# IlyaGrebnov/libbsc

Measured on AMD Instinct MI355X. Metric: MB/s compress (BWT+QLFC) on 64 MiB blocks, higher is better.
Workload: dtype u8; 1 GPU; 1 x 64 MiB synth-text-v1 block(s) per step, bsc_compress(lzp off, sorter=1, coder=1); 5 GPU context(s) x 4 block(s) in flight per GPU, 20 coder threads; block_bytes=67108864, sorter=BWT, coder=QLFC static (-e1), parallelism=block-parallel x1, compressed_bytes_rank0=15277890

## Files before the change

include/bscgpu.h:

```cpp
#ifndef BSCGPU_H
#define BSCGPU_H

#include <stddef.h>
#include <stdint.h>

#if defined(__GNUC__)
#define BSCGPU_API __attribute__((visibility("default")))
#else
#define BSCGPU_API
#endif

#ifdef __cplusplus
extern "C" {
#endif

typedef struct bscgpu_ctx bscgpu_ctx;

BSCGPU_API int bscgpu_device_count(void);

BSCGPU_API int  bscgpu_create(bscgpu_ctx** ctx, int device, int64_t max_n);
BSCGPU_API void bscgpu_destroy(bscgpu_ctx* ctx);

BSCGPU_API int64_t bscgpu_arena_bytes(const bscgpu_ctx* ctx);

// ... 160 lines not shown
};
typedef struct bscgpu_kstat {
    double   ms;
    uint64_t launches;
    uint64_t bytes;
    uint64_t records;
} bscgpu_kstat;
BSCGPU_API void bscgpu_profile_enable(bscgpu_ctx* ctx, int on);
BSCGPU_API void bscgpu_profile_reset(bscgpu_ctx* ctx);
BSCGPU_API int  bscgpu_profile_get(bscgpu_ctx* ctx, bscgpu_kstat* stats );
BSCGPU_API int  bscgpu_profile_scatter_launches(bscgpu_ctx* ctx, double* ms, uint64_t* records, int max);
BSCGPU_API int  bscgpu_last_stage_ms(bscgpu_ctx* ctx, double* out6);

BSCGPU_API const char* bscgpu_last_error(const bscgpu_ctx* ctx);

enum { BSCGPU_OPT_RS_ONESWEEP = 1, BSCGPU_CNT_OS_RETRIES = 2, BSCGPU_OPT_DC_PACKED_STREAM = 4,
       BSCGPU_CNT_DC_REPLAYS = 5, BSCGPU_CNT_DC_LAST_FAIL = 6, BSCGPU_CNT_DC_AVG_UNDECIDED = 7, BSCGPU_CNT_DC_HIST_EXTENDED = 8,
       BSCGPU_OPT_BATCH_FRONT = 9, BSCGPU_CNT_BATCH_FRONT_PASSES = 10, BSCGPU_CNT_BATCH_L_PASSES = 11,
       BSCGPU_OPT_DEVICE_RC = 12, BSCGPU_CNT_DEVICE_RC_BLOCKS = 13,
       BSCGPU_OPT_BATCH_MODEL = 14, BSCGPU_CNT_BATCH_MODEL_PASSES = 15, BSCGPU_CNT_BATCH_MODEL_DECLINED = 16,
       BSCGPU_OPT_BATCH_MODEL_FAST = 17, BSCGPU_CNT_BATCH_FAST_PASSES = 18, BSCGPU_CNT_BATCH_FAST_DECLINED = 19,
       BSCGPU_OPT_BWT_FOLD = 20, BSCGPU_CNT_BWT_FOLDED = 21,
       BSCGPU_OPT_BATCH_MODEL_SEGMENTS = 22, BSCGPU_CNT_BATCH_SEGMENTS = 23, BSCGPU_CNT_BATCH_SEG_RERUNS = 24,
       BSCGPU_CNT_BATCH_SEG_HOST_BLOCKS = 25, BSCGPU_CNT_DC_DCAP = 26 };
enum { BSCGPU_DC_FAIL_AVG = 2, BSCGPU_DC_FAIL_HIST = 4, BSCGPU_DC_FAIL_CAP = 8, BSCGPU_DC_FAIL_REPLAY = 16 };
BSCGPU_API int bscgpu_option_set(bscgpu_ctx* ctx, int key, int value);
BSCGPU_API int bscgpu_option_get(bscgpu_ctx* ctx, int key);
enum { BSCGPU_PCNT_DEVICE_MODEL_BLOCKS = 1, BSCGPU_PCNT_REDONE_ON_HOST_MODEL = 2, BSCGPU_PCNT_DEVICE_MODEL_LZP_BLOCKS = 3 };
BSCGPU_API long long bscgpu_process_counter(int key);

BSCGPU_API int bscgpu_dispatch_device(int slot, int nphys);
BSCGPU_API int bscgpu_dispatch_pick(int nphys, int ctx_per_dev, const int* users, const unsigned char* usable, unsigned start);

#ifdef __cplusplus
}
#endif
#endif
```

libbsc_amd/csrc/device/context.hip:

```cpp
#include "dev_common.h"
#include "dma_copy.h"
#include <sys/mman.h>
#include <system_error>
#include <thread>
#include <vector>
#include <chrono>
#include <cstdio>
#include <cstdlib>
#include <cstring>
#include <functional>
#include <memory>
#include <mutex>

int ctx_fail(bscgpu_ctx* c, int code, const char* what, hipError_t e)
{
    if (c) {
        char buf[512];
        snprintf(buf, sizeof buf, "%s: %s", what, e == hipSuccess ? "failed" : hipGetErrorString(e));
        c->err = buf;
    }
    return code;
}

bool ctx_timing_on() { static const bool on = getenv("BSCGPU_TIMING") != nullptr; return on; }
// ... 134 lines not shown
    if (hipGetDeviceCount(&n) != hipSuccess) return 0;
    return n;
}

#ifndef ARENA_ALIGN
#define ARENA_ALIGN 256
#endif
extern "C" int bscgpu_create(bscgpu_ctx** out, int device, int64_t max_n)
{
    if (!out || max_n < 0 || max_n >= 0x7fffffffll) return BSC_BAD_PARAMETER;
    *out = nullptr;
    CtxTimer tm_all("bscgpu_create");
    int ndev = 0;
    if (hipGetDeviceCount(&ndev) != hipSuccess || ndev <= 0) return BSC_GPU_NOT_SUPPORTED;
    if (device < 0 || device >= ndev) return BSC_BAD_PARAMETER;
    devcoder_warm_tables();
    if (hipSetDevice(device) != hipSuccess) return BSC_GPU_ERROR;
    if (!getenv("BSCGPU_SPIN")) { (void)hipSetDeviceFlags(hipDeviceScheduleBlockingSync); (void)hipGetLastError(); }

    bscgpu_ctx* c = new bscgpu_ctx();
    { CtxTimer tm("  first HIP call on this thread"); (void)hipFree(nullptr); }
    c->device = device;
    c->max_n  = max_n;
    { const char* e = getenv("BSC_PS13"); c->dc_p13 = (e && e[0] == '0') ? 0 : 1; }
    { const char* e = getenv("BSC_BWT_FOLD"); if (e && e[0] >= '0' && e[0] <= '2' && !e[1]) c->bwt_fold = e[0] - '0'; }
    memset(c->kstat, 0, sizeof c->kstat);
    auto tm_streams = std::make_unique<CtxTimer>("  streams + events");
    if (hipStreamCreateWithFlags(&c->stream, hipStreamNonBlocking) != hipSuccess) { delete c; return BSC_GPU_ERROR; }
    if (hipEventCreateWithFlags(&c->sync_ev, hipEventBlockingSync | hipEventDisableTiming) != hipSuccess) { hipStreamDestroy(c->stream); delete c; return BSC_GPU_ERROR; }
    if (hipStreamCreateWithFlags(&c->copy_stream, hipStreamNonBlocking) != hipSuccess) { hipEventDestroy(c->sync_ev); hipStreamDestroy(c->stream); delete c; return BSC_GPU_ERROR; }

    tm_streams.reset();
    const size_t N = align_up((size_t)max_n + 4096, 4096);
    struct Carve { void** p; size_t bytes; size_t lead; };
    Carve carve[] = {
        {(void**)&c->dT,      N + 128, 64},
        {(void**)&c->dL,      N + 64, 0},
        {(void**)&c->kA,      8 * N, 0}, {(void**)&c->kB, 8 * N, 0},
        {(void**)&c->vA,      4 * N, 0}, {(void**)&c->vB, 4 * N, 0},
        {(void**)&c->SA,      4 * N, 0}, {(void**)&c->ISA, 4 * N + 64, 0},
        {(void**)&c->cpos[0], 4 * N, 0}, {(void**)&c->cpos[1], 4 * N, 0},
        {(void**)&c->csa[0],  4 * N, 0}, {(void**)&c->csa[1],  4 * N, 0},
        {(void**)&c->cgrp[0], 4 * N, 0}, {(void**)&c->cgrp[1], 4 * N, 0},
        {(void**)&c->flags,   N + 64, 0},
        {(void**)&c->counts,  (size_t)256 * MAX_CHUNKS * 4, 0},
        {(void**)&c->rowtot,  256 * 4, 0},
// ... 106 lines not shown
{
    if (!c) return;
    memset(c->kstat, 0, sizeof c->kstat);
    c->scatter_log.clear();
}
extern "C" int bscgpu_profile_get(bscgpu_ctx* c, bscgpu_kstat* stats)
{
    if (!c || !stats) return BSC_BAD_PARAMETER;
    memcpy(stats, c->kstat, sizeof c->kstat);
    return BSC_NO_ERROR;
}
extern "C" int bscgpu_profile_scatter_launches(bscgpu_ctx* c, double* ms, uint64_t* records, int max)
{
    if (!c) return 0;
    int cnt = (int)c->scatter_log.size();
    int from = cnt > max ? cnt - max : 0;
    for (int i = from; i < cnt; ++i) { ms[i - from] = c->scatter_log[i].ms; records[i - from] = c->scatter_log[i].records; }
    return cnt - from;
}
extern "C" int bscgpu_option_set(bscgpu_ctx* c, int key, int value)
{
    if (!c) return BSC_BAD_PARAMETER;
    if (key == BSCGPU_OPT_RS_ONESWEEP && value >= 0 && value <= 3 && (value == 0 || c->os_available)) { const int old = c->os_mode; c->os_mode = value; return old; }
    if (key == BSCGPU_OPT_DC_PACKED_STREAM && (value == 0 || value == 1)) { const int old = c->dc_p13; c->dc_p13 = value; return old; }
    if (key == BSCGPU_OPT_BATCH_FRONT && (value == 0 || value == 1)) { const int old = c->batch_front; c->batch_front = value; return old; }
    if (key == BSCGPU_OPT_DEVICE_RC && (value == 0 || value == 1)) { const int old = c->device_rc; c->device_rc = value; return old; }
    if (key == BSCGPU_OPT_BATCH_MODEL && (value == 0 || value == 1)) { const int old = c->batch_model; c->batch_model = value; return old; }
    if (key == BSCGPU_OPT_BATCH_MODEL_FAST && (value == 0 || value == 1)) { const int old = c->batch_model_fast; c->batch_model_fast = value; return old; }
    if (key == BSCGPU_OPT_BATCH_MODEL_SEGMENTS && (value == 0 || value == 1)) { const int old = c->batch_model_segments; c->batch_model_segments = value; return old; }
    if (key == BSCGPU_OPT_BWT_FOLD && value >= 0 && value <= 2) { const int old = c->bwt_fold; c->bwt_fold = value; return old; }
    return BSC_BAD_PARAMETER;
}
extern "C" int bscgpu_option_get(bscgpu_ctx* c, int key)
{
    if (!c) return BSC_BAD_PARAMETER;
    if (key == BSCGPU_OPT_RS_ONESWEEP) return c->os_mode;
    if (key == BSCGPU_CNT_OS_RETRIES) return c->os_retries;
    if (key == BSCGPU_OPT_DC_PACKED_STREAM) return c->dc_p13;
    if (key == BSCGPU_CNT_DC_REPLAYS) return c->dc_replays;
    if (key == BSCGPU_CNT_DC_LAST_FAIL) return c->dc_last_fail;
    if (key == BSCGPU_CNT_DC_AVG_UNDECIDED) return c->dc_avg_und;
    if (key == BSCGPU_CNT_DC_HIST_EXTENDED) return c->dc_hist_ext;
    if (key == BSCGPU_OPT_BATCH_FRONT) return c->batch_front;
    if (key == BSCGPU_CNT_BATCH_FRONT_PASSES) return c->cnt_front_passes;
    if (key == BSCGPU_CNT_BATCH_L_PASSES) return c->cnt_l_passes;
    if (key == BSCGPU_OPT_DEVICE_RC) return c->device_rc;
    if (key == BSCGPU_CNT_DEVICE_RC_BLOCKS) return c->cnt_device_rc;
    if (key == BSCGPU_OPT_BATCH_MODEL) return c->batch_model;
    if (key == BSCGPU_CNT_BATCH_MODEL_PASSES) return c->cnt_model_passes;
    if (key == BSCGPU_CNT_BATCH_MODEL_DECLINED) return c->cnt_model_declined;
    if (key == BSCGPU_OPT_BATCH_MODEL_FAST) return c->batch_model_fast;
    if (key == BSCGPU_CNT_BATCH_FAST_PASSES) return c->cnt_model_fast_passes;
    if (key == BSCGPU_CNT_BATCH_FAST_DECLINED) return c->cnt_model_fast_declined;
    if (key == BSCGPU_OPT_BATCH_MODEL_SEGMENTS) return c->batch_model_segments;
    if (key == BSCGPU_CNT_BATCH_SEGMENTS) return c->cnt_seg;
    if (key == BSCGPU_CNT_BATCH_SEG_RERUNS) return c->cnt_seg_reruns;
    if (key == BSCGPU_CNT_BATCH_SEG_HOST_BLOCKS) return c->cnt_seg_host_blocks;
    if (key == BSCGPU_CNT_DC_DCAP) { const int64_t v = devcoder_dcap(c); return v > 0x7fffffff ? 0x7fffffff : (int)v; }
    if (key == BSCGPU_OPT_BWT_FOLD) return c->bwt_fold;
    if (key == BSCGPU_CNT_BWT_FOLDED) return c->cnt_bwt_folded;
    return BSC_BAD_PARAMETER;
}
extern "C" int bscgpu_last_stage_ms(bscgpu_ctx* c, double* out6)
{
    if (!c || !out6) return BSC_BAD_PARAMETER;
// ... 92 lines not shown
```

libbsc_amd/csrc/device/dev_common.h:

```cpp
#pragma once
#include <hip/hip_runtime.h>
#include <stdint.h>
#include <stddef.h>
#include <string>
#include <vector>

#include "../../../include/bscgpu.h"

typedef unsigned long long u64;
typedef unsigned int       u32;
typedef unsigned short     u16;
typedef unsigned char      u8;

#define BSC_NO_ERROR                0
#define BSC_BAD_PARAMETER          -1
#define BSC_NOT_ENOUGH_MEMORY      -2
#define BSC_NOT_COMPRESSIBLE       -3
#define BSC_NOT_SUPPORTED          -4
#define BSC_DATA_CORRUPT           -6
#define BSC_GPU_ERROR              -7
#define BSC_GPU_NOT_SUPPORTED      -8
#define BSC_GPU_NOT_ENOUGH_MEMORY  -9

constexpr int   WG          = 256;
// ... 80 lines not shown
    int  device_rc = 0;
    int  cnt_device_rc = 0;
    int  batch_model = 0;
    int  cnt_model_passes = 0, cnt_model_declined = 0;
    int  batch_model_fast = 0;
    int  cnt_model_fast_passes = 0, cnt_model_fast_declined = 0;
    int  batch_model_segments = 0;
    int  cnt_seg = 0, cnt_seg_reruns = 0, cnt_seg_host_blocks = 0;
    u16* model_host[2] = {nullptr, nullptr};
    size_t model_host_entries = 0;
    bool model_host_failed = false;
    u64* wc_sink = nullptr;
    int  num_cus = 256;
    int  os_mode = 0;
    u32* os_agg = nullptr;
    u32* os_zero = nullptr;
    u32  os_tiles_cap = 0;
    u32  os_pass_stride = 0;
    u32  os_batch_words = 0;
    u32  os_epoch = 0;
    bool os_check_pending = false;
    bool os_available = true;
    int  os_retries = 0;
    int  dc_p13 = 1;
    bool os_gave_up = false;
    int  bwt_fold = 1;
    int  cnt_bwt_folded = 0;
    bool fold_lds_set = false;
    u32* hscal  = nullptr;
    u64* hscal64 = nullptr;
    u64* hadler = nullptr;
    u64* hsplit = nullptr;
    HostSlot slots[MAX_SLOTS];
    int      nslots = 0;
    DevCoder* dc = nullptr;
    bool     dc_alloc_failed = false;
    int      dc_last_fail = 0;
    int      dc_replays = 0;
    int      dc_avg_und = 0;
    int      dc_hist_ext = 0;

    bool         prof        = false;
    bscgpu_kstat kstat[BSCGPU_K_COUNT];
    std::vector<ScatterLaunch> scatter_log;
    struct Pending { hipEvent_t a, b; int kind; u64 bytes; u64 records; };
    std::vector<Pending> pending;
    std::vector<hipEvent_t> event_pool;
    double       stage_ms[6] = {0, 0, 0, 0, 0, 0};

    std::string  err;
};

int  ctx_fail(bscgpu_ctx* c, int code, const char* what, hipError_t e);
bool ctx_timing_on();
struct CtxTimer {
    const char* what; double t0; bool on;
    explicit CtxTimer(const char* w);
    ~CtxTimer();
};
hipError_t ctx_sync(bscgpu_ctx* c);
#define HIP_TRY(ctx, expr)                                                         \
    do { hipError_t _e = (expr);                                                   \
// ... 145 lines not shown
```

libbsc_amd/csrc/device/devcoder.hip:

```cpp
#include "dev_common.h"
#include "dma_copy.h"
#include <thread>
#include <system_error>
#include "devcoder_model.h"
#include "../host/qlfc.h"
#include <cstdio>
#include <cstdlib>
#include <cstring>
#include <deque>
#include <vector>
#include <type_traits>

using namespace dcm;

#ifndef DC_XCD_RANGES
#define DC_XCD_RANGES 0
#endif
__device__ __forceinline__ u32 dc_virtual_block() {
    if (!DC_XCD_RANGES) return blockIdx.x;
    return (blockIdx.x & 7u) * (gridDim.x >> 3) + (blockIdx.x >> 3);
}

constexpr int DC_WCH_MAX  = 4096;
constexpr u32 DC_SIGMASK  = 0x7ffu;
constexpr int DC_ROWS     = 1088;

enum { DM_FAIL = 0, DM_NTYPES, DM_NROUNDS, DM_AVG_UND, DM_REPLAYS, DM_D0, DM_D1, DM_D2, DM_D3, DM_HIST_EXT , DM_P13_OVER , DM_COUNT = 16 };
enum { FAIL_AVG = BSCGPU_DC_FAIL_AVG, FAIL_HIST = BSCGPU_DC_FAIL_HIST, FAIL_CAP = BSCGPU_DC_FAIL_CAP, FAIL_REPLAY = BSCGPU_DC_FAIL_REPLAY };

struct DcSub { u32 nb; u32 first[9]; u32 maxr[8]; };
struct DcRowBins { u16 lo1, hi1, lo2, hi2; };

struct DevCoder {
    size_t Mcap = 0, Dcap = 0;
    char*  arena = nullptr; size_t arena_bytes = 0;
    u64 *key_ch = nullptr, *key_ch_s = nullptr, *key_sr = nullptr, *key_sr_s = nullptr, *key_sn = nullptr, *key_sn_s = nullptr;
    u32 *inv_ch = nullptr, *inv_sr = nullptr, *inv_sn = nullptr;
    u8  *ge32 = nullptr;
    u32 *doff[4] = {nullptr, nullptr, nullptr, nullptr};
    u16 *events[4] = {nullptr, nullptr, nullptr, nullptr};
    u32 *pos[4] = {nullptr, nullptr, nullptr, nullptr};
    u16 *V[4] = {nullptr, nullptr, nullptr, nullptr};
    size_t nch_cap = 0;
    u16 *ps[2] = {nullptr, nullptr};
    u32 *cnt = nullptr, *rowtot = nullptr, *rowstart = nullptr , *wdec = nullptr, *wdecoff = nullptr;
    u16 *elo = nullptr, *ehi = nullptr, *S = nullptr;
    u32 *present = nullptr; u8 *rounds = nullptr; u32 *meta = nullptr; u32 *poff = nullptr;
    DcRowBins* rowbins = nullptr;
    u16* sink = nullptr;
    u8  *tab_rank = nullptr, *tab_run = nullptr;
    ModelParams* mp = nullptr;
    ModelParams* mp_fast = nullptr;
    struct DcFrag* frag = nullptr;
    u32 *hmeta = nullptr;
    char*  batch_arena = nullptr; size_t batch_bytes = 0; bool batch_alloc_failed = false;
    u16 *esub[4] = {nullptr, nullptr, nullptr, nullptr};
    u8  *sub_maxr = nullptr; u32 *poff_tab = nullptr;
    u32 *sub_und = nullptr, *sub_dec = nullptr, *seg_run = nullptr;
    hipEvent_t seg_ev[2] = {nullptr, nullptr};
};

__device__ __forceinline__ u32 dc_sb_of(u32 j, const DcSub& S)
{
    u32 sb = 0;
#pragma unroll
    for (int b = 1; b < 8; ++b) if ((u32)b < S.nb && j >= S.first[b]) sb = b;
    return sb;
}
__device__ __forceinline__ u32 dc_maxr_pack(const DcSub& S)
// ... 615 lines not shown
#pragma unroll
    for (u32 x = 0; x < 8; ++x) {
        const u32 id = (w[x >> 1] >> (16u * (x & 1u))) & 0xffffu;
        if (id != prev && k0 + x < E) ev[k0 + x] |= (u16)DC_ROWMARK;
        prev = id;
    }
}

__device__ __forceinline__ int dc_class_first_row(int cls)
{
    return cls == CLS_RF ? TAU_RF : cls == CLS_RE ? TAU_RE : cls == CLS_RM ? TAU_RM : cls == CLS_RP ? TAU_RP : cls == CLS_NF ? TAU_NF
         : cls == CLS_NE ? TAU_NE : cls == CLS_NM ? TAU_NM : cls == CLS_NM2 ? TAU_NM2 : DC_ROWS;
}

constexpr int DC_EVAL_WAVES = 4;
constexpr int DC_EVAL_LDS_WAVE = 2 * 64 * DC_EROW;
constexpr int DC_EVAL_LDS = DC_EVAL_WAVES * (DC_EVAL_LDS_WAVE + NUM_CLS * 4 + NUM_CLS * (int)sizeof(Rates));
__device__ __forceinline__ void dc_wave_sync()
{
    __builtin_amdgcn_fence(__ATOMIC_ACQ_REL, "wavefront");
    __builtin_amdgcn_wave_barrier();
}

template <bool WRITE>
__global__ __launch_bounds__(64 * DC_EVAL_WAVES) void dc_eval_wave_kernel(DcEvalAll A, const ModelParams* __restrict__ mp, const u32* __restrict__ meta,
                                                          u16* __restrict__ elo_all, u16* __restrict__ ehi_all, const u16* __restrict__ Sv_all, u32* __restrict__ tdbg)
{
#if DC_EVAL_TIMING
    const u64 t_begin = wall_clock64();
    u32 slow_batches = 0;
#endif
    extern __shared__ __attribute__((aligned(16))) u8 dc_eval_lds[];
    const u32 wv = threadIdx.x >> 6, lane = threadIdx.x & 63u;
    u8* const sin = dc_eval_lds + wv * DC_EVAL_LDS_WAVE;
    u8* const sout = sin + 64 * DC_EROW;
    u32* const sclsend = reinterpret_cast<u32*>(dc_eval_lds + DC_EVAL_WAVES * DC_EVAL_LDS_WAVE) + wv * NUM_CLS;
    Rates* const srate = reinterpret_cast<Rates*>(dc_eval_lds + DC_EVAL_WAVES * (DC_EVAL_LDS_WAVE + NUM_CLS * 4)) + wv * NUM_CLS;
    const u32 gw = blockIdx.x * DC_EVAL_WAVES + wv;
    if (meta[DM_FAIL] != 0u || gw >= A.wstart[4]) return;
    int jb = 0;
#pragma unroll
    for (int q = 1; q < 4; ++q) if (gw >= A.wstart[q]) jb = q;
    const DcEvalJob J = A.job[jb];
    if (lane < (u32)NUM_CLS) {
        srate[lane] = mp->rates[lane][J.fam];
        sclsend[lane] = J.rowstart[dc_class_first_row((int)lane + 1)];
    }
    dc_wave_sync();
    u16* const elo = elo_all + A.cstart[jb];
    u16* const ehi = ehi_all + A.cstart[jb];
    const u16* const Sv = Sv_all + A.cstart[jb];
    u16* const Vout = A.V[jb];
    const u32 wave = gw - A.wstart[jb];
    const u32 c = wave * 64 + lane;
    const u32 EV = A.ev;
    const u64 k0 = (u64)c * EV;
    const bool mine = k0 < J.E;
    const u32 k1 = mine ? (u32)((k0 + EV < J.E) ? k0 + EV : J.E) : 0u;
    const u32 crow = lane >> 3, ccol = lane & 7u;
    const u64 wave_k0 = (u64)wave * 64 * EV;

    u32 cls = 0, clsend = 0, prev = 0xffffu;
    int init = mp->init[0];
    int lo = init, hi = init;
    Rates R = srate[0];
    if (mine) {
        while (cls + 1 < (u32)NUM_CLS && sclsend[cls] <= (u32)k0) ++cls;
        clsend = sclsend[cls];
        R = srate[cls];
        init = mp->init[cls];
        prev = (k0 > 0) ? ((u32)J.events[k0 - 1] & DC_SIGMASK) : 0xffffu;
        if (WRITE) { lo = Sv[c]; hi = lo; } else { lo = mp->vmin[cls][J.fam]; hi = mp->vmax[cls][J.fam]; }
    }
    auto fetch = [&](u32 b, uint4* q) {
#pragma unroll
        for (int i = 0; i < 8; ++i) {
            const u64 kk = wave_k0 + (u64)(8 * i + crow) * EV + (u64)b * DC_EB + ccol * 8;
            const u64 ka = kk < J.E ? kk : 0ull;
            const uint4 val = *reinterpret_cast<const uint4*>(J.events + ka);
            q[i].x = val.x; q[i].y = val.y; q[i].z = val.z; q[i].w = val.w;
        }
    };
    auto store_out = [&](u32 b) {
#pragma unroll
        for (int i = 0; i < 8; ++i) {
            const u64 kk = wave_k0 + (u64)(8 * i + crow) * EV + (u64)b * DC_EB + ccol * 8;
            *reinterpret_cast<uint4*>(kk < J.E ? Vout + kk : A.sink + lane * 8) = *reinterpret_cast<const uint4*>(sout + (8 * i + crow) * DC_EROW + ccol * 16);
        }
    };
    uint4 nxt[8];
    fetch(0, nxt);
    const u32 NB = EV / DC_EB;
    for (u32 b = 0; b < NB; ++b) {
#pragma unroll
        for (int i = 0; i < 8; ++i) *reinterpret_cast<uint4*>(sin + (8 * i + crow) * DC_EROW + ccol * 16) = nxt[i];
        dc_wave_sync();
        if (WRITE && b > 0) store_out(b - 1);
        fetch(b + 1 < NB ? b + 1 : b, nxt);
        const u32 kb = (u32)k0 + b * DC_EB;
        if (mine && kb < k1) {
            const u8* myrow = sin + lane * DC_EROW;
            u8* orow = sout + lane * DC_EROW;
            const u32 lim = k1 < clsend ? k1 : clsend;
            if (kb + DC_EB <= lim) {
                const int c0 = R.t0 * R.a0 + R.r0, c1 = R.t1 * R.a1 + R.r1;
#pragma unroll
                for (int g8 = 0; g8 < 8; ++g8) {
                    const uint4 q = *reinterpret_cast<const uint4*>(myrow + g8 * 16);
                    const u32 wds[4] = {q.x, q.y, q.z, q.w};
                    u32 outw[4] = {0, 0, 0, 0};
#pragma unroll
                    for (int x = 0; x < 8; ++x) {
                        const u32 e = (wds[x >> 1] >> (16 * (x & 1))) & 0xffffu;
                        const u32 sigm = e & (DC_SIGMASK | DC_ROWMARK);
                        if (sigm != prev) { lo = init; hi = init; }
                        prev = e & DC_SIGMASK;
                        const bool b1 = (e & 0x800u) != 0u;
                        const int Cc = b1 ? c1 : c0, Aa = b1 ? R.a1 : R.a0;
                        if (WRITE) outw[x >> 1] |= (u32)lo << (16 * (x & 1));
                        lo += (Cc - __mul24(lo, Aa)) >> 12;
                        if (!WRITE) hi += (Cc - __mul24(hi, Aa)) >> 12;
                    }
                    if (WRITE) *reinterpret_cast<uint4*>(orow + g8 * 16) = make_uint4(outw[0], outw[1], outw[2], outw[3]);
                }
            } else {
#if DC_EVAL_TIMING
                ++slow_batches;
#endif
                const u32 cnt = (k1 - kb < (u32)DC_EB) ? k1 - kb : (u32)DC_EB;
                for (u32 x = 0; x < cnt; ++x) {
                    const u32 k = kb + x;
                    while (k >= clsend && cls + 1 < (u32)NUM_CLS) { ++cls; clsend = sclsend[cls]; R = srate[cls]; init = mp->init[cls]; }
                    const u32 e = *reinterpret_cast<const u16*>(myrow + 2 * x);
                    if ((e & (DC_SIGMASK | DC_ROWMARK)) != prev) { lo = init; hi = init; }
                    prev = e & DC_SIGMASK;
                    const u32 bt = (e >> 11) & 1u;
                    if (WRITE) *reinterpret_cast<u16*>(orow + 2 * x) = (u16)lo;
                    lo = step(lo, bt, R);
                    if (!WRITE) hi = step(hi, bt, R);
                }
            }
        }
        dc_wave_sync();
    }
    if (WRITE) store_out(NB - 1);
    if (!WRITE && mine) { elo[c] = (u16)lo; ehi[c] = (u16)hi; }
#if DC_EVAL_TIMING
    {
        u32 sb = slow_batches;
        for (int d = 32; d >= 1; d >>= 1) { const u32 o = (u32)__shfl_xor((int)sb, d, 64); sb = sb > o ? sb : o; }
        if (lane == 0) { tdbg[3 * gw] = (u32)(t_begin & 0xffffffffu); tdbg[3 * gw + 1] = (u32)(wall_clock64() - t_begin); tdbg[3 * gw + 2] = sb | ((u32)jb << 16); }
    }
#endif
}

__device__ __forceinline__ bool dc_chunk_continues(const DcEvalJob& J, u32 c, u32 EV)
{
    if (c == 0) return false;
    const u32 k0 = c * EV;
    u32 row = dc_find_row(J.rowstart, k0);
    if (J.rowstart[row] == k0) return false;
    const u32 e1 = J.events[k0];
    return ((((u32)J.events[k0 - 1] ^ e1) & DC_SIGMASK) | (e1 & DC_ROWMARK)) == 0;
}

__global__ __launch_bounds__(WG) void dc_eval_b_kernel(DcEvalAll A, const ModelParams* __restrict__ mp, u32* __restrict__ meta,
                                                       const u16* __restrict__ elo_all, const u16* __restrict__ ehi_all, u16* __restrict__ Sv_all)
{
    if (meta[DM_FAIL] != 0u) return;
// ... 382 lines not shown
int64_t devcoder_dcap(const bscgpu_ctx* c) { return (int64_t)dc_capacity_decisions(c->max_n); }

int devcoder_ensure(bscgpu_ctx* c)
{
    if (c->dc) return BSC_NO_ERROR;
    if (c->dc_alloc_failed) return BSC_NOT_SUPPORTED;
    if (getenv("BSC_DEVCODER_FAIL_ALLOC")) { c->dc_alloc_failed = true; return BSC_NOT_SUPPORTED; }
    CtxTimer tm("devcoder_ensure (arena, tables)");
    DevCoder* d = new DevCoder();
    d->Mcap = dc_capacity_runs(c->max_n); d->Dcap = dc_capacity_decisions(c->max_n);
    const size_t M = d->Mcap + 64, D = d->Dcap + 64, NCH = d->Dcap / DC_EV + 16;
    struct Carve { void** p; size_t bytes; };
    Carve carve[] = {
        {(void**)&d->key_ch, 8 * M}, {(void**)&d->key_ch_s, 8 * M}, {(void**)&d->key_sr, 8 * M}, {(void**)&d->key_sr_s, 8 * M},
        {(void**)&d->key_sn, 8 * M}, {(void**)&d->key_sn_s, 8 * M},
        {(void**)&d->inv_ch, 4 * M}, {(void**)&d->inv_sr, 4 * M}, {(void**)&d->inv_sn, 4 * M}, {(void**)&d->ge32, M},
        {(void**)&d->doff[0], 4 * M}, {(void**)&d->doff[1], 4 * M}, {(void**)&d->doff[2], 4 * M}, {(void**)&d->doff[3], 4 * M},
        {(void**)&d->events[0], 2 * D}, {(void**)&d->events[1], 2 * D}, {(void**)&d->events[2], 2 * D}, {(void**)&d->events[3], 2 * D},
        {(void**)&d->pos[0], 4 * D}, {(void**)&d->pos[1], 4 * D}, {(void**)&d->pos[2], 4 * D}, {(void**)&d->pos[3], 4 * D},
        {(void**)&d->V[0], 2 * D}, {(void**)&d->V[1], 2 * D}, {(void**)&d->V[2], 2 * D}, {(void**)&d->V[3], 2 * D},
        {(void**)&d->ps[0], 2 * D}, {(void**)&d->ps[1], 2 * D},
        {(void**)&d->cnt, (size_t)DC_ROWS * DC_WCH_MAX * 4}, {(void**)&d->rowtot, DC_ROWS * 4}, {(void**)&d->rowstart, 6 * (DC_ROWS + 8) * 4},
        {(void**)&d->wdec, (DC_WCH_MAX + 8) * 4}, {(void**)&d->wdecoff, (DC_WCH_MAX + 8) * 4},
        {(void**)&d->elo, 2 * 4 * NCH}, {(void**)&d->ehi, 2 * 4 * NCH}, {(void**)&d->S, 2 * 4 * NCH},
        {(void**)&d->present, (size_t)DC_KIND_WORDS * 4}, {(void**)&d->rounds, 256},
        {(void**)&d->meta, DM_COUNT * 4}, {(void**)&d->poff, 16 * 4}, {(void**)&d->frag, (M / 64 + 64) * 2 * sizeof(DcFrag)},
        {(void**)&d->tab_rank, 32768}, {(void**)&d->tab_run, 8192}, {(void**)&d->mp, sizeof(ModelParams)}, {(void**)&d->mp_fast, sizeof(ModelParams)},
        {(void**)&d->rowbins, DC_ROWS * sizeof(DcRowBins)}, {(void**)&d->sink, 4096},
    };
    size_t total = 0;
    for (auto& cv : carve) total += dc_align(cv.bytes);
    if (hipMalloc((void**)&d->arena, total) != hipSuccess) { (void)hipGetLastError(); delete d; c->dc_alloc_failed = true; return BSC_NOT_SUPPORTED; }
    d->arena_bytes = total; d->nch_cap = NCH;
    size_t off = 0;
    for (auto& cv : carve) { *cv.p = d->arena + off; off += dc_align(cv.bytes); }
    if (hipHostMalloc((void**)&d->hmeta, 64 * 4, hipHostMallocDefault) != hipSuccess) { (void)hipGetLastError(); hipFree(d->arena); delete d; c->dc_alloc_failed = true; return BSC_NOT_SUPPORTED; }
    const ModelParams& mp = dc_model_static();
    const ModelParams& mpf = dc_model_fast();
    if (hipFuncSetAttribute((const void*)dc_eval_wave_kernel<false>, hipFuncAttributeMaxDynamicSharedMemorySize, DC_EVAL_LDS) != hipSuccess ||
        hipFuncSetAttribute((const void*)dc_eval_wave_kernel<true>, hipFuncAttributeMaxDynamicSharedMemorySize, DC_EVAL_LDS) != hipSuccess) {
        (void)hipFree(d->arena); (void)hipHostFree(d->hmeta); delete d;
        return ctx_fail(c, BSC_GPU_ERROR, "device coder: LDS attribute", hipSuccess);
    }
    static DcRowBins rowbins[DC_ROWS];
    static const bool rowbins_ok = dc_build_rowbins(rowbins);
    if (!rowbins_ok) { (void)hipFree(d->arena); (void)hipHostFree(d->hmeta); delete d; return ctx_fail(c, BSC_GPU_ERROR, "device coder: bin layout", hipSuccess); }
    const bschost::QlfcTables& QT = bschost::qlfc_tables();
// ... 16 lines not shown
static void dc_launch_partition(bscgpu_ctx* c, DevCoder* d, const u64* items, u32 m, const SB& S, int job, u32 ignoreX)
{
    const DcGeom g = dc_geom(m);
    const u32 grid = (g.W + WAVES - 1) / WAVES;
    u32* rowstart = d->rowstart + (DC_ROWS + 8) * job;
    prof_begin(c, BSCGPU_K_DC_PART, (u64)m * 8, m);
    hipLaunchKernelGGL((dc_part_count_kernel<SIDES, SB>), dim3(grid), dim3(WG), 0, c->stream, items, g, S, d->rowbins, d->cnt, d->wdec);
    hipLaunchKernelGGL(dc_scan_rows_kernel, dim3(DC_ROWS), dim3(WG), 0, c->stream, d->cnt, g.W, d->rowtot);
    hipLaunchKernelGGL(dc_scan_misc_kernel, dim3(1), dim3(WG), 0, c->stream, d->rowtot, rowstart, d->wdec, g.W, d->wdecoff, d->meta, job, (u32)d->Dcap);
    if constexpr (SCATTER)
        hipLaunchKernelGGL((dc_part_scatter_kernel<SIDES, SB>), dim3(grid), dim3(WG), 0, c->stream, items, g, S, d->meta, d->cnt, rowstart,
                           d->wdecoff, ignoreX, d->events[job], d->pos[job], d->doff[job], d->esub[job]);
    else
        hipLaunchKernelGGL((dc_doff_kernel<SIDES, SB>), dim3(grid), dim3(WG), 0, c->stream, items, g, S, d->meta, d->wdecoff, d->doff[job]);
    prof_end(c);
}

static void dc_note_block(bscgpu_ctx* c, const DevCoder* d)
{
    c->dc_last_fail = (int)d->hmeta[DM_FAIL];
    c->dc_replays = (int)d->hmeta[DM_REPLAYS];
    c->dc_avg_und = (int)d->hmeta[DM_AVG_UND];
    c->dc_hist_ext = (int)d->hmeta[DM_HIST_EXT];
}

struct DcDown { void* dst; const void* src; size_t bytes; };
static int dc_meta_down(bscgpu_ctx* c, DevCoder* d, const DcDown& also)
{
    HIP_TRY(c, hipGetLastError());
    HIP_TRY(c, hipMemcpyAsync(d->hmeta, d->meta, DM_COUNT * 4, hipMemcpyDeviceToHost, c->stream));
    if (also.dst) HIP_TRY(c, hipMemcpyAsync(also.dst, also.src, also.bytes, hipMemcpyDeviceToHost, c->stream));
    HIP_TRY(c, ctx_sync(c));
    prof_collect(c);
    dc_note_block(c, d);
    return d->hmeta[DM_FAIL] != 0 ? BSC_NOT_SUPPORTED : BSC_NO_ERROR;
}

static int dc_ps_wait(bscgpu_ctx* c, int psbuf)
{
    if (c->ps_guard[psbuf & 1]) HIP_TRY(c, hipStreamWaitEvent(c->stream, c->ps_guard[psbuf & 1], 0));
    for (int b = 0; b < 8; ++b)
        if (c->ps_guard_sig[psbuf & 1][b] && dma_wait(c->ps_guard_sig[psbuf & 1][b]) != 0)
            return ctx_fail(c, BSC_GPU_ERROR, "device coder: the stream buffer's previous copy-out failed", hipSuccess);
    return BSC_NO_ERROR;
}

// ... 10 lines not shown

static int dc_eval(bscgpu_ctx* c, DevCoder* d, const u32 E[4], const int fam[4], const ModelParams* mp, bool tab)
{
    DcEvalAll A;
    A.wstart[0] = 0; A.cstart[0] = 0; A.sink = d->sink;
    A.ev = eval_chunk_events((u64)E[0] + E[1] + E[2] + E[3]);
    for (int job = 0; job < 4; ++job) {
        A.job[job].events = d->events[job]; A.job[job].E = E[job]; A.job[job].rowstart = d->rowstart + (DC_ROWS + 8) * job;
        A.job[job].fam = fam[job];
        A.V[job] = d->V[job];
        const u32 nch = (E[job] + A.ev - 1) / A.ev;
        A.wstart[job + 1] = A.wstart[job] + (nch + 63) / 64;
        A.cstart[job + 1] = A.cstart[job] + (nch + 63) / 64 * 64;
    }
    if (A.cstart[4] > 4 * d->nch_cap) return ctx_fail(c, BSC_GPU_ERROR, "device coder: chunk table too small", hipSuccess);
    prof_begin(c, BSCGPU_K_DC_EVAL, (u64)(E[0] + E[1] + E[2] + E[3]) * 6, (u64)E[0] + E[1] + E[2] + E[3]);
    if (A.wstart[4] > 0) {
        hipLaunchKernelGGL(dc_mark_rows_kernel, dim3((4 * DC_ROWS + WG - 1) / WG), dim3(WG), 0, c->stream, A);
        if (tab) {
            DcMarkAll K; u32 emax = 0;
            for (int job = 0; job < 4; ++job) { K.events[job] = d->events[job]; K.esub[job] = d->esub[job]; K.E[job] = E[job]; if (E[job] > emax) emax = E[job]; }
            hipLaunchKernelGGL(dc_mark_chains_kernel, dim3((emax + 8 * WG - 1) / (8 * WG), 4), dim3(WG), 0, c->stream, K, d->meta);
        }
        hipLaunchKernelGGL(dc_eval_wave_kernel<false>, dim3((A.wstart[4] + DC_EVAL_WAVES - 1) / DC_EVAL_WAVES), dim3(64 * DC_EVAL_WAVES), DC_EVAL_LDS, c->stream, A, mp, d->meta, d->elo, d->ehi, (const u16*)nullptr, d->cnt);
        hipLaunchKernelGGL(dc_eval_b_kernel, dim3((A.cstart[4] + WG - 1) / WG), dim3(WG), 0, c->stream, A, mp, d->meta, d->elo, d->ehi, d->S);
        hipLaunchKernelGGL(dc_eval_wave_kernel<true>, dim3((A.wstart[4] + DC_EVAL_WAVES - 1) / DC_EVAL_WAVES), dim3(64 * DC_EVAL_WAVES), DC_EVAL_LDS, c->stream, A, mp, d->meta, (u16*)nullptr, (u16*)nullptr, d->S, d->cnt + 3 * 4096);
    }
    prof_end(c);
    return BSC_NO_ERROR;
}

template <class SB>
static int dc_static_run(bscgpu_ctx* c, DevCoder* d, const SB& S, const u8* dsym, const u8* drank, const u32* dstart, const u8* ge32, u32 m, u32 n,
                         bool ctx_open, int psbuf, int64_t expect, u32* poff_host, u16* dbg, int* packed_out, u32* D_out)
{
    const u32 gm = (m + WG - 1) / WG;
    const u32 gm8 = (gm + 7u) / 8u * 8u;
    if (!ctx_open) prof_begin(c, BSCGPU_K_DC_CTX, (u64)m * 40, m);
    hipLaunchKernelGGL(dc_items_kernel<SB>, dim3(gm), dim3(WG), 0, c->stream, dsym, drank, dstart, ge32, m, n, S, d->key_ch);
    prof_end(c);
    RadixPass top; top.shift = 56; top.bits = 8;
    int in_alt = 0;
    int rc = radix_sort_passes(c, d->key_ch, d->key_ch_s, nullptr, nullptr, m, &top, 1, &in_alt, d->inv_ch);
    if (rc < 0) return rc;
    prof_begin(c, BSCGPU_K_DC_CTX, (u64)m * 40, m);
    hipLaunchKernelGGL(dc_ctx_kernel<SB>, dim3(gm8), dim3(WG), 0, c->stream, d->key_ch, d->key_ch_s, d->inv_ch, m, S, d->tab_rank, d->tab_run,
                       d->key_sr, d->key_sn, d->present, d->meta);
    hipLaunchKernelGGL(dc_setup_kernel<SB>, dim3(1), dim3(WG), 0, c->stream, d->present, S, d->rounds, d->meta);
    prof_end(c);
// ... 429 lines not shown
```

libbsc_amd/gpu.py:

```python
import ctypes as C

import numpy as np

from . import _native as N


class GpuError(RuntimeError):
    def __init__(self, code, msg=""):
        super().__init__(f"bscgpu error {code}: {msg}")
        self.code = code


def _dptr(t):
    if isinstance(t, int):
        return C.c_void_p(t)
    import torch
    torch.cuda.current_stream(t.device).synchronize()
    return C.c_void_p(t.data_ptr())


class GpuContext:

    def __init__(self, device=0, max_n=64 << 20):
        self.L = N.lib()
# ... 292 lines not shown
        inp, isz = self._pack(blocks)
        ds = np.zeros(max(isz.size, 1), np.int32)
        total = self._check(int(self.L.bscgpu_decompress_batch_sizes(N.np_ptr(inp), N.np_ptr(isz), isz.size, N.np_ptr(ds))))
        out = torch.empty(max(total, 1), dtype=torch.uint8, device=f"cuda:{self.device}")
        results = np.zeros(max(isz.size, 1), np.int32)
        self._check(self.L.bscgpu_decompress_batch_device(self.h, N.np_ptr(inp), N.np_ptr(isz), isz.size, _dptr(out), total,
                                                          N.np_ptr(results), features))
        offs = [0]
        for b in range(isz.size):
            offs.append(offs[-1] + int(ds[b]))
        return out[:total], offs, [int(x) for x in results[:isz.size]]

    def pipe(self, depth=2, reuse_outputs=False):
        return Pipe(self, depth, reuse_outputs)

    OPT_RS_ONESWEEP, CNT_OS_RETRIES, OPT_DC_PACKED_STREAM = 1, 2, 4
    OPT_BATCH_FRONT, CNT_BATCH_FRONT_PASSES, CNT_BATCH_L_PASSES = 9, 10, 11
    OPT_DEVICE_RC, CNT_DEVICE_RC_BLOCKS = 12, 13
    OPT_BATCH_MODEL, CNT_BATCH_MODEL_PASSES, CNT_BATCH_MODEL_DECLINED = 14, 15, 16
    OPT_BATCH_MODEL_FAST, CNT_BATCH_FAST_PASSES, CNT_BATCH_FAST_DECLINED = 17, 18, 19
    OPT_BWT_FOLD, CNT_BWT_FOLDED = 20, 21
    OPT_BATCH_MODEL_SEGMENTS, CNT_BATCH_SEGMENTS, CNT_BATCH_SEG_RERUNS, CNT_BATCH_SEG_HOST_BLOCKS, CNT_DC_DCAP = 22, 23, 24, 25, 26
    CNT_DC_REPLAYS, CNT_DC_LAST_FAIL, CNT_DC_AVG_UNDECIDED, CNT_DC_HIST_EXTENDED = 5, 6, 7, 8
    DC_FAIL_AVG, DC_FAIL_HIST, DC_FAIL_CAP, DC_FAIL_REPLAY = 2, 4, 8, 16

    def option_set(self, key, value):
        return self._check(self.L.bscgpu_option_set(self.h, key, value))

    def option_get(self, key):
        return self._check(self.L.bscgpu_option_get(self.h, key))

    def profile(self, on=True):
        self.L.bscgpu_profile_enable(self.h, 1 if on else 0)

    def profile_reset(self):
        self.L.bscgpu_profile_reset(self.h)

    def profile_get(self):
        arr = (N.KStat * len(N.K_NAMES))()
        self.L.bscgpu_profile_get(self.h, arr)
        return {N.K_NAMES[i]: dict(ms=arr[i].ms, launches=int(arr[i].launches), bytes=int(arr[i].bytes),
                                   records=int(arr[i].records)) for i in range(len(N.K_NAMES))}

    def scatter_launches(self, max_n=4096):
        ms = (C.c_double * max_n)()
        rec = (C.c_uint64 * max_n)()
# ... 249 lines not shown
```

Measured before the change: 6036 MB/s.

## Record bracket-convergence prefix in eval pass and rewalk only that prefix

The first evaluation pass now tracks per wave how many leading batches still carry an unresolved lo/hi bracket. Once every lane converges it switches to a single-state walk and records that batch count. The second (write) pass reads this prefix and rewalks only those batches instead of the whole chunk, skipping redundant event processing and stores. It adds per-wave ballots, atomic counters and a prefix buffer, and relies on outputs beyond the prefix already being correct from the first pass.

```diff
diff --git a/include/bscgpu.h b/include/bscgpu.h
--- a/include/bscgpu.h
+++ b/include/bscgpu.h
@@ -206,7 +206,8 @@
        BSCGPU_OPT_BATCH_MODEL_FAST = 17, BSCGPU_CNT_BATCH_FAST_PASSES = 18, BSCGPU_CNT_BATCH_FAST_DECLINED = 19,
        BSCGPU_OPT_BWT_FOLD = 20, BSCGPU_CNT_BWT_FOLDED = 21,
        BSCGPU_OPT_BATCH_MODEL_SEGMENTS = 22, BSCGPU_CNT_BATCH_SEGMENTS = 23, BSCGPU_CNT_BATCH_SEG_RERUNS = 24,
-       BSCGPU_CNT_BATCH_SEG_HOST_BLOCKS = 25, BSCGPU_CNT_DC_DCAP = 26 };
+       BSCGPU_CNT_BATCH_SEG_HOST_BLOCKS = 25, BSCGPU_CNT_DC_DCAP = 26,
+       BSCGPU_OPT_DC_EVAL_PREFIX = 27, BSCGPU_CNT_DC_EVAL_BATCHES = 28, BSCGPU_CNT_DC_EVAL_REWALKED = 29 };
 enum { BSCGPU_DC_FAIL_AVG = 2, BSCGPU_DC_FAIL_HIST = 4, BSCGPU_DC_FAIL_CAP = 8, BSCGPU_DC_FAIL_REPLAY = 16 };
 BSCGPU_API int bscgpu_option_set(bscgpu_ctx* ctx, int key, int value);
 BSCGPU_API int bscgpu_option_get(bscgpu_ctx* ctx, int key);
diff --git a/libbsc_amd/csrc/device/context.hip b/libbsc_amd/csrc/device/context.hip
--- a/libbsc_amd/csrc/device/context.hip
+++ b/libbsc_amd/csrc/device/context.hip
@@ -180,6 +180,7 @@
     { CtxTimer tm("  first HIP call on this thread"); (void)hipFree(nullptr); }
     c->device = device;
     c->max_n  = max_n;
+    { const char* e = getenv("BSC_DC_EVAL_PREFIX"); c->dc_eval_prefix = (e && e[0] == '0') ? 0 : 1; }
     { const char* e = getenv("BSC_PS13"); c->dc_p13 = (e && e[0] == '0') ? 0 : 1; }
     { const char* e = getenv("BSC_BWT_FOLD"); if (e && e[0] >= '0' && e[0] <= '2' && !e[1]) c->bwt_fold = e[0] - '0'; }
     memset(c->kstat, 0, sizeof c->kstat);
@@ -332,6 +333,7 @@
 {
     if (!c) return BSC_BAD_PARAMETER;
     if (key == BSCGPU_OPT_RS_ONESWEEP && value >= 0 && value <= 3 && (value == 0 || c->os_available)) { const int old = c->os_mode; c->os_mode = value; return old; }
+    if (key == BSCGPU_OPT_DC_EVAL_PREFIX && (value == 0 || value == 1)) { const int old = c->dc_eval_prefix; c->dc_eval_prefix = value; return old; }
     if (key == BSCGPU_OPT_DC_PACKED_STREAM && (value == 0 || value == 1)) { const int old = c->dc_p13; c->dc_p13 = value; return old; }
     if (key == BSCGPU_OPT_BATCH_FRONT && (value == 0 || value == 1)) { const int old = c->batch_front; c->batch_front = value; return old; }
     if (key == BSCGPU_OPT_DEVICE_RC && (value == 0 || value == 1)) { const int old = c->device_rc; c->device_rc = value; return old; }
@@ -351,6 +353,9 @@
     if (key == BSCGPU_CNT_DC_LAST_FAIL) return c->dc_last_fail;
     if (key == BSCGPU_CNT_DC_AVG_UNDECIDED) return c->dc_avg_und;
     if (key == BSCGPU_CNT_DC_HIST_EXTENDED) return c->dc_hist_ext;
+    if (key == BSCGPU_OPT_DC_EVAL_PREFIX) return c->dc_eval_prefix;
+    if (key == BSCGPU_CNT_DC_EVAL_BATCHES) return c->dc_eval_batches;
+    if (key == BSCGPU_CNT_DC_EVAL_REWALKED) return c->dc_eval_rewalked;
     if (key == BSCGPU_OPT_BATCH_FRONT) return c->batch_front;
     if (key == BSCGPU_CNT_BATCH_FRONT_PASSES) return c->cnt_front_passes;
     if (key == BSCGPU_CNT_BATCH_L_PASSES) return c->cnt_l_passes;
diff --git a/libbsc_amd/csrc/device/dev_common.h b/libbsc_amd/csrc/device/dev_common.h
--- a/libbsc_amd/csrc/device/dev_common.h
+++ b/libbsc_amd/csrc/device/dev_common.h
@@ -126,6 +126,7 @@
     bool os_check_pending = false;
     bool os_available = true;
     int  os_retries = 0;
+    int  dc_eval_prefix = 1;
     int  dc_p13 = 1;
     bool os_gave_up = false;
     int  bwt_fold = 1;
@@ -142,6 +143,7 @@
     int      dc_last_fail = 0;
     int      dc_replays = 0;
     int      dc_avg_und = 0;
+    int      dc_eval_batches = 0, dc_eval_rewalked = 0;
     int      dc_hist_ext = 0;
 
     bool         prof        = false;
diff --git a/libbsc_amd/csrc/device/devcoder.hip b/libbsc_amd/csrc/device/devcoder.hip
--- a/libbsc_amd/csrc/device/devcoder.hip
+++ b/libbsc_amd/csrc/device/devcoder.hip
@@ -25,7 +25,8 @@
 constexpr u32 DC_SIGMASK  = 0x7ffu;
 constexpr int DC_ROWS     = 1088;
 
-enum { DM_FAIL = 0, DM_NTYPES, DM_NROUNDS, DM_AVG_UND, DM_REPLAYS, DM_D0, DM_D1, DM_D2, DM_D3, DM_HIST_EXT , DM_P13_OVER , DM_COUNT = 16 };
+enum { DM_FAIL = 0, DM_NTYPES, DM_NROUNDS, DM_AVG_UND, DM_REPLAYS, DM_D0, DM_D1, DM_D2, DM_D3, DM_HIST_EXT , DM_P13_OVER ,
+       DM_EVAL_BATCHES , DM_EVAL_REWALK , DM_COUNT = 16 };
 enum { FAIL_AVG = BSCGPU_DC_FAIL_AVG, FAIL_HIST = BSCGPU_DC_FAIL_HIST, FAIL_CAP = BSCGPU_DC_FAIL_CAP, FAIL_REPLAY = BSCGPU_DC_FAIL_REPLAY };
 
 struct DcSub { u32 nb; u32 first[9]; u32 maxr[8]; };
@@ -45,6 +46,7 @@
     u16 *ps[2] = {nullptr, nullptr};
     u32 *cnt = nullptr, *rowtot = nullptr, *rowstart = nullptr , *wdec = nullptr, *wdecoff = nullptr;
     u16 *elo = nullptr, *ehi = nullptr, *S = nullptr;
+    u32 *eprefix = nullptr;
     u32 *present = nullptr; u8 *rounds = nullptr; u32 *meta = nullptr; u32 *poff = nullptr;
     DcRowBins* rowbins = nullptr;
     u16* sink = nullptr;
@@ -706,9 +708,10 @@
     __builtin_amdgcn_wave_barrier();
 }
 
-template <bool WRITE>
-__global__ __launch_bounds__(64 * DC_EVAL_WAVES) void dc_eval_wave_kernel(DcEvalAll A, const ModelParams* __restrict__ mp, const u32* __restrict__ meta,
-                                                          u16* __restrict__ elo_all, u16* __restrict__ ehi_all, const u16* __restrict__ Sv_all, u32* __restrict__ tdbg)
+template <bool REWALK>
+__global__ __launch_bounds__(64 * DC_EVAL_WAVES) void dc_eval_wave_kernel(DcEvalAll A, const ModelParams* __restrict__ mp, u32* __restrict__ meta,
+                                                          u16* __restrict__ elo_all, u16* __restrict__ ehi_all, const u16* __restrict__ Sv_all,
+                                                          u32* __restrict__ prefix, u32 full, u32* __restrict__ tdbg)
 {
 #if DC_EVAL_TIMING
     const u64 t_begin = wall_clock64();
@@ -722,6 +725,14 @@
     Rates* const srate = reinterpret_cast<Rates*>(dc_eval_lds + DC_EVAL_WAVES * (DC_EVAL_LDS_WAVE + NUM_CLS * 4)) + wv * NUM_CLS;
     const u32 gw = blockIdx.x * DC_EVAL_WAVES + wv;
     if (meta[DM_FAIL] != 0u || gw >= A.wstart[4]) return;
+    const u32 EV = A.ev;
+    const u32 NB = EV / DC_EB;
+    u32 nwalk = NB;
+    if (REWALK) {
+        if (!full) { const u32 rec = (u32)__builtin_amdgcn_readfirstlane((int)prefix[gw]); nwalk = rec < NB ? rec : NB; }
+        if (lane == 0) { atomicAdd(&meta[DM_EVAL_BATCHES], NB); atomicAdd(&meta[DM_EVAL_REWALK], nwalk); }
+        if (nwalk == 0) return;
+    }
     int jb = 0;
 #pragma unroll
     for (int q = 1; q < 4; ++q) if (gw >= A.wstart[q]) jb = q;
@@ -737,7 +748,6 @@
     u16* const Vout = A.V[jb];
     const u32 wave = gw - A.wstart[jb];
     const u32 c = wave * 64 + lane;
-    const u32 EV = A.ev;
     const u64 k0 = (u64)c * EV;
     const bool mine = k0 < J.E;
     const u32 k1 = mine ? (u32)((k0 + EV < J.E) ? k0 + EV : J.E) : 0u;
@@ -754,7 +764,7 @@
         R = srate[cls];
         init = mp->init[cls];
         prev = (k0 > 0) ? ((u32)J.events[k0 - 1] & DC_SIGMASK) : 0xffffu;
-        if (WRITE) { lo = Sv[c]; hi = lo; } else { lo = mp->vmin[cls][J.fam]; hi = mp->vmax[cls][J.fam]; }
+        if (REWALK) { lo = Sv[c]; hi = lo; } else { lo = mp->vmin[cls][J.fam]; hi = mp->vmax[cls][J.fam]; }
     }
     auto fetch = [&](u32 b, uint4* q) {
 #pragma unroll
@@ -772,63 +782,79 @@
             *reinterpret_cast<uint4*>(kk < J.E ? Vout + kk : A.sink + lane * 8) = *reinterpret_cast<const uint4*>(sout + (8 * i + crow) * DC_EROW + ccol * 16);
         }
     };
+    auto walk = [&](u32 kb, auto both) {
+        constexpr bool BOTH = decltype(both)::value;
+        const u8* myrow = sin + lane * DC_EROW;
+        u8* orow = sout + lane * DC_EROW;
+        const u32 lim = k1 < clsend ? k1 : clsend;
+        if (kb + DC_EB <= lim) {
+            const int c0 = R.t0 * R.a0 + R.r0, c1 = R.t1 * R.a1 + R.r1;
+#pragma unroll
+            for (int g8 = 0; g8 < 8; ++g8) {
+                const uint4 q = *reinterpret_cast<const uint4*>(myrow + g8 * 16);
+                const u32 wds[4] = {q.x, q.y, q.z, q.w};
+                u32 outw[4] = {0, 0, 0, 0};
+#pragma unroll
+                for (int x = 0; x < 8; ++x) {
+                    const u32 e = (wds[x >> 1] >> (16 * (x & 1))) & 0xffffu;
+                    const u32 sigm = e & (DC_SIGMASK | DC_ROWMARK);
+                    if (sigm != prev) { lo = init; if (BOTH) hi = init; }
+                    prev = e & DC_SIGMASK;
+                    const bool b1 = (e & 0x800u) != 0u;
+                    const int Cc = b1 ? c1 : c0, Aa = b1 ? R.a1 : R.a0;
+                    outw[x >> 1] |= (u32)lo << (16 * (x & 1));
+                    lo += (Cc - __mul24(lo, Aa)) >> 12;
+                    if (BOTH) hi += (Cc - __mul24(hi, Aa)) >> 12;
+                }
+                *reinterpret_cast<uint4*>(orow + g8 * 16) = make_uint4(outw[0], outw[1], outw[2], outw[3]);
+            }
+        } else {
+#if DC_EVAL_TIMING
+            ++slow_batches;
+#endif
+            const u32 cnt = (k1 - kb < (u32)DC_EB) ? k1 - kb : (u32)DC_EB;
+            for (u32 x = 0; x < cnt; ++x) {
+                const u32 k = kb + x;
+                while (k >= clsend && cls + 1 < (u32)NUM_CLS) { ++cls; clsend = sclsend[cls]; R = srate[cls]; init = mp->init[cls]; }
+                const u32 e = *reinterpret_cast<const u16*>(myrow + 2 * x);
+                if ((e & (DC_SIGMASK | DC_ROWMARK)) != prev) { lo = init; if (BOTH) hi = init; }
+                prev = e & DC_SIGMASK;
+                const u32 bt = (e >> 11) & 1u;
+                *reinterpret_cast<u16*>(orow + 2 * x) = (u16)lo;
+                lo = step(lo, bt, R);
+                if (BOTH) hi = step(hi, bt, R);
+            }
+        }
+    };
     uint4 nxt[8];
     fetch(0, nxt);
-    const u32 NB = EV / DC_EB;
-    for (u32 b = 0; b < NB; ++b) {
+    bool bracket = !REWALK;
+    u64 single = 0;
+    u32 unmet_batches = 0;
+    for (u32 b = 0; b < nwalk; ++b) {
 #pragma unroll
         for (int i = 0; i < 8; ++i) *reinterpret_cast<uint4*>(sin + (8 * i + crow) * DC_EROW + ccol * 16) = nxt[i];
         dc_wave_sync();
-        if (WRITE && b > 0) store_out(b - 1);
-        fetch(b + 1 < NB ? b + 1 : b, nxt);
+        if (b > 0) store_out(b - 1);
+        fetch(b + 1 < nwalk ? b + 1 : b, nxt);
         const u32 kb = (u32)k0 + b * DC_EB;
-        if (mine && kb < k1) {
-            const u8* myrow = sin + lane * DC_EROW;
-            u8* orow = sout + lane * DC_EROW;
-            const u32 lim = k1 < clsend ? k1 : clsend;
-            if (kb + DC_EB <= lim) {
-                const int c0 = R.t0 * R.a0 + R.r0, c1 = R.t1 * R.a1 + R.r1;
-#pragma unroll
-                for (int g8 = 0; g8 < 8; ++g8) {
-                    const uint4 q = *reinterpret_cast<const uint4*>(myrow + g8 * 16);
-                    const u32 wds[4] = {q.x, q.y, q.z, q.w};
-                    u32 outw[4] = {0, 0, 0, 0};
-#pragma unroll
-                    for (int x = 0; x < 8; ++x) {
-                        const u32 e = (wds[x >> 1] >> (16 * (x & 1))) & 0xffffu;
-                        const u32 sigm = e & (DC_SIGMASK | DC_ROWMARK);
-                        if (sigm != prev) { lo = init; hi = init; }
-                        prev = e & DC_SIGMASK;
-                        const bool b1 = (e & 0x800u) != 0u;
-                        const int Cc = b1 ? c1 : c0, Aa = b1 ? R.a1 : R.a0;
-                        if (WRITE) outw[x >> 1] |= (u32)lo << (16 * (x & 1));
-                        lo += (Cc - __mul24(lo, Aa)) >> 12;
-                        if (!WRITE) hi += (Cc - __mul24(hi, Aa)) >> 12;
-                    }
-                    if (WRITE) *reinterpret_cast<uint4*>(orow + g8 * 16) = make_uint4(outw[0], outw[1], outw[2], outw[3]);
-                }
-            } else {
-#if DC_EVAL_TIMING
-                ++slow_batches;
-#endif
-                const u32 cnt = (k1 - kb < (u32)DC_EB) ? k1 - kb : (u32)DC_EB;
-                for (u32 x = 0; x < cnt; ++x) {
-                    const u32 k = kb + x;
-                    while (k >= clsend && cls + 1 < (u32)NUM_CLS) { ++cls; clsend = sclsend[cls]; R = srate[cls]; init = mp->init[cls]; }
-                    const u32 e = *reinterpret_cast<const u16*>(myrow + 2 * x);
-                    if ((e & (DC_SIGMASK | DC_ROWMARK)) != prev) { lo = init; hi = init; }
-                    prev = e & DC_SIGMASK;
-                    const u32 bt = (e >> 11) & 1u;
-                    if (WRITE) *reinterpret_cast<u16*>(orow + 2 * x) = (u16)lo;
-                    lo = step(lo, bt, R);
-                    if (!WRITE) hi = step(hi, bt, R);
-                }
-            }
-        }
+        const bool act = mine && kb < k1;
+        if (!REWALK && bracket) {
+            const u32 e0 = *reinterpret_cast<const u16*>(sin + lane * DC_EROW);
+            const bool unmet = act && lo != hi && (e0 & (DC_SIGMASK | DC_ROWMARK)) == prev;
+            if (__ballot(unmet) != 0ull) unmet_batches = b + 1;
+            else { bracket = false; single = __ballot(act); }
+        }
+        if (!REWALK && bracket) { if (act) walk(kb, std::true_type()); }
+        else                    { if (act) walk(kb, std::false_type()); }
         dc_wave_sync();
     }
-    if (WRITE) store_out(NB - 1);
-    if (!WRITE && mine) { elo[c] = (u16)lo; ehi[c] = (u16)hi; }
+    store_out(nwalk - 1);
+    if (!REWALK) {
+        if ((single >> lane) & 1ull) hi = lo;
+        if (mine) { elo[c] = (u16)lo; ehi[c] = (u16)hi; }
+        if (lane == 0) prefix[gw] = unmet_batches;
+    }
 #if DC_EVAL_TIMING
     {
         u32 sb = slow_batches;
@@ -1257,7 +1283,7 @@
         {(void**)&d->ps[0], 2 * D}, {(void**)&d->ps[1], 2 * D},
         {(void**)&d->cnt, (size_t)DC_ROWS * DC_WCH_MAX * 4}, {(void**)&d->rowtot, DC_ROWS * 4}, {(void**)&d->rowstart, 6 * (DC_ROWS + 8) * 4},
         {(void**)&d->wdec, (DC_WCH_MAX + 8) * 4}, {(void**)&d->wdecoff, (DC_WCH_MAX + 8) * 4},
-        {(void**)&d->elo, 2 * 4 * NCH}, {(void**)&d->ehi, 2 * 4 * NCH}, {(void**)&d->S, 2 * 4 * NCH},
+        {(void**)&d->elo, 2 * 4 * NCH}, {(void**)&d->ehi, 2 * 4 * NCH}, {(void**)&d->S, 2 * 4 * NCH}, {(void**)&d->eprefix, (4 * NCH / 64 + 8) * 4},
         {(void**)&d->present, (size_t)DC_KIND_WORDS * 4}, {(void**)&d->rounds, 256},
         {(void**)&d->meta, DM_COUNT * 4}, {(void**)&d->poff, 16 * 4}, {(void**)&d->frag, (M / 64 + 64) * 2 * sizeof(DcFrag)},
         {(void**)&d->tab_rank, 32768}, {(void**)&d->tab_run, 8192}, {(void**)&d->mp, sizeof(ModelParams)}, {(void**)&d->mp_fast, sizeof(ModelParams)},
@@ -1320,6 +1346,8 @@
     c->dc_replays = (int)d->hmeta[DM_REPLAYS];
     c->dc_avg_und = (int)d->hmeta[DM_AVG_UND];
     c->dc_hist_ext = (int)d->hmeta[DM_HIST_EXT];
+    c->dc_eval_batches = (int)d->hmeta[DM_EVAL_BATCHES];
+    c->dc_eval_rewalked = (int)d->hmeta[DM_EVAL_REWALK];
 }
 
 struct DcDown { void* dst; const void* src; size_t bytes; };
@@ -1376,9 +1404,11 @@
             for (int job = 0; job < 4; ++job) { K.events[job] = d->events[job]; K.esub[job] = d->esub[job]; K.E[job] = E[job]; if (E[job] > emax) emax = E[job]; }
             hipLaunchKernelGGL(dc_mark_chains_kernel, dim3((emax + 8 * WG - 1) / (8 * WG), 4), dim3(WG), 0, c->stream, K, d->meta);
         }
-        hipLaunchKernelGGL(dc_eval_wave_kernel<false>, dim3((A.wstart[4] + DC_EVAL_WAVES - 1) / DC_EVAL_WAVES), dim3(64 * DC_EVAL_WAVES), DC_EVAL_LDS, c->stream, A, mp, d->meta, d->elo, d->ehi, (const u16*)nullptr, d->cnt);
+        const dim3 wgrid((A.wstart[4] + DC_EVAL_WAVES - 1) / DC_EVAL_WAVES), wblock(64 * DC_EVAL_WAVES);
+        const u32 full = c->dc_eval_prefix ? 0u : 1u;
+        hipLaunchKernelGGL(dc_eval_wave_kernel<false>, wgrid, wblock, DC_EVAL_LDS, c->stream, A, mp, d->meta, d->elo, d->ehi, (const u16*)nullptr, d->eprefix, 0u, d->cnt);
         hipLaunchKernelGGL(dc_eval_b_kernel, dim3((A.cstart[4] + WG - 1) / WG), dim3(WG), 0, c->stream, A, mp, d->meta, d->elo, d->ehi, d->S);
-        hipLaunchKernelGGL(dc_eval_wave_kernel<true>, dim3((A.wstart[4] + DC_EVAL_WAVES - 1) / DC_EVAL_WAVES), dim3(64 * DC_EVAL_WAVES), DC_EVAL_LDS, c->stream, A, mp, d->meta, (u16*)nullptr, (u16*)nullptr, d->S, d->cnt + 3 * 4096);
+        hipLaunchKernelGGL(dc_eval_wave_kernel<true>, wgrid, wblock, DC_EVAL_LDS, c->stream, A, mp, d->meta, (u16*)nullptr, (u16*)nullptr, d->S, d->eprefix, full, d->cnt + 3 * 4096);
     }
     prof_end(c);
     return BSC_NO_ERROR;
diff --git a/libbsc_amd/gpu.py b/libbsc_amd/gpu.py
--- a/libbsc_amd/gpu.py
+++ b/libbsc_amd/gpu.py
@@ -338,6 +338,7 @@
     OPT_BWT_FOLD, CNT_BWT_FOLDED = 20, 21
     OPT_BATCH_MODEL_SEGMENTS, CNT_BATCH_SEGMENTS, CNT_BATCH_SEG_RERUNS, CNT_BATCH_SEG_HOST_BLOCKS, CNT_DC_DCAP = 22, 23, 24, 25, 26
     CNT_DC_REPLAYS, CNT_DC_LAST_FAIL, CNT_DC_AVG_UNDECIDED, CNT_DC_HIST_EXTENDED = 5, 6, 7, 8
+    OPT_DC_EVAL_PREFIX, CNT_DC_EVAL_BATCHES, CNT_DC_EVAL_REWALKED = 27, 28, 29
     DC_FAIL_AVG, DC_FAIL_HIST, DC_FAIL_CAP, DC_FAIL_REPLAY = 2, 4, 8, 16
 
     def option_set(self, key, value):
```

New measurement: 6096 MB/s (median of 6 runs). Within noise of the previous version (+1.0%).
